# Ben-Bussch/Lunar_Module_Ascent_Trajectory_Optimiser

Measured on AMD Instinct MI355X. Metric: solved ascent NLPs/sec (N=200 collocation nodes), higher is better.
Workload: dtype f64; 1 GPU; BASELINE.json configs[2]: 4096-NLP Isp x dry-mass sweep (64x64, Isp 300-320 s, dry mass 2345-2545 kg), N=200 nodes, backward Euler (reference NODES=2), DCOST applied (the script's MV move penalty 1e-05, Launch_Optimiser.py:99, as an l1 term: the model the reference declares); move_penalty=True, batch_per_gpu=4096, global_batch=4096, n_nodes=200, parallelism=problem-sharded x1, gather only, converged=4096, of=4096

## Files before the change

### lunar_module_ascent_trajectory_optimiser_amd/csrc/ascent_persist.hip

```cpp
#include <hip/hip_runtime.h>

#pragma clang fp contract(on)

#include <cstdio>
#include <cstdlib>

#include "ascent.h"
#include "ascent_device.hpp"
#include "ascent_tile.hpp"
#include "ascent_persist.hpp"
#include "ascent_persist_dev.hpp"

using namespace ascent;

namespace {


ASC_DEV void start_move(double *w, int Kp, int k, double u, double up, bool warm, double dcw) {
  const double dl = u - up, eps = warm ? 1e-4 : 1e-2;
  w[(R_IT + O_LU) * Kp + k] = 0.0;
  w[(R_IT + O_PP) * Kp + k] = fmax(dl, 0.0) + eps;
  w[(R_IT + O_PN) * Kp + k] = fmax(-dl, 0.0) + eps;
  w[(R_IT + O_ZP) * Kp + k] = dcw;
  w[(R_IT + O_ZN) * Kp + k] = dcw;
// ... 354 lines not shown
    P.rd = fmax(P.rd, fmax(fabs(t.dcw - lu - kp.zpp), fabs(t.dcw + lu - kp.zpn)));
  }
  const double cs = SCHEME == 1 ? 0.5 * t.dt : t.dt;
  double fl[7], lt[7];
  ASC_UNROLL
  for (int i = 0; i < 7; i++) lt[i] = SCHEME == 1 ? l[i] + ln[i] : l[i];
  fzt_lambda<FORM>(kp.G, lt, fl);
  double r[7];
  ASC_UNROLL
  for (int i = 0; i < 7; i++) {
    r[i] = (FORM == 1 && i == IA) ? l[i] - cs * fl[i] : l[i] - cs * fl[i] - ln[i];
    P.rth -= t.hT * kp.F[i] * l[i];
    P.l1 += fabs(l[i]);
  }
  r[IA] += kp.dza;
  r[IM] += kp.dzm;
  if (k == K - 1) {
    const Scal &stt = t.stt;
    double z[7];
    ASC_UNROLL
    for (int i = 0; i < 7; i++) z[i] = in[(O_Z + i) * Kp + k];
    if constexpr (TERM == 2) {
      const Terminal tt = terminal_eval_any(d, z);
      double g4[4];
      terminal_grad_any(tt, stt.nu1, stt.nu2, g4);
      r[IX] += g4[0]; r[IY] += g4[1]; r[IVX] += g4[2]; r[IVY] += g4[3];
    } else {
      const Terminal tt = terminal_eval(d, z);
      r[IX] += stt.nu3 * tt.e3g[0] + stt.nu1 * tt.g1g[0];
      r[IY] += stt.nu3 * tt.e3g[1] + stt.nu1 * tt.g1g[1];
      r[IVX] += stt.nu3 * tt.e3g[2] + stt.nu2 * tt.g2g[0];
      r[IVY] += stt.nu3 * tt.e3g[3] + stt.nu2 * tt.g2g[1];
    }
  }
  ASC_UNROLL
  for (int i = 0; i < 7; i++) P.rd = fmax(P.rd, fabs(r[i]));
  double ruv = (FORM == 1 ? -0.5 * d.aub * l[IA] : -t.be * l[IW]) - kp.zb4 + kp.zb5;
  if constexpr (MP) ruv += lu - lun;
  P.rd = fmax(P.rd, fabs(ruv));
}

template <int SCHEME, int FORM, int MP = 0, int TERM = 0>
ASC_DEV void trial_node(const Der &d, int K, int Kp, int k, const NodeIn &n, const NodeIn &dn, const TrialCtx &t, bool live,
                        double *in, Part &P) {
  TrialKeep kp;
  trial_primal<SCHEME, FORM, MP, TERM>(d, K, Kp, k, n, dn, t, live, in, P, kp);
  double l[7], ln[7];
  ASC_UNROLL
  for (int i = 0; i < 7; i++) { l[i] = n.l[i] + t.alpha * dn.l[i]; ln[i] = n.ln[i] + t.alpha * dn.ln[i]; }
  const double lu = MP ? n.lu + t.alpha * dn.lu : 0.0, lun = MP ? n.lun + t.alpha * dn.lun : 0.0;
  trial_dual<SCHEME, FORM, MP, TERM>(d, K, Kp, k, kp, l, ln, lu, lun, t, live, in, P);
}


template <int SCHEME, int FORM, int MP = 0, int TERM = 0, int WIDE = 0>
__global__ __launch_bounds__(WAVE) void p_solve(const ascent_params *params, long batch, PGeo g, double *ws, int max_iter, double tol) {
  using L = Lay<MP>;
  constexpr int NS = L::NS, NIT = L::NIT, R_ST = L::R_ST, R_KA = L::R_KA, R_K0 = L::R_K0, NROWS = L::NROWS;
  constexpr int S_G = L::S_G, S_E = L::S_E, S_H = L::S_H, S_F = L::S_F, S_C = L::S_C, S_RZ = L::S_RZ, S_GT = L::S_GT, S_SC = L::S_SC;
  constexpr int RL = NS;
  static_assert(FORM == 0 || SCHEME == 0, "the v1 formulation is restated with backward Euler");
  __shared__ double stage[L::S_ROWS * LDW];
  __shared__ double outb[L::OUT_ROWS * LDW];
  __shared__ double lds_t[NPW][NS][NS];
  __shared__ double lds_d[NPW][3][8];
  __shared__ double lsc[NPW][NSCAL];
  __shared__ double lds_c[NPW][8];
  constexpr int CHN = WIDE ? 64 : CH;
  const int lane = threadIdx.x, grp = lane >> 4, role = lane & 15;
  const int nl = WIDE ? lane : role;
  const int cbase = WIDE ? 0 : grp * 16;
  const long p = WIDE ? (long)blockIdx.x : (long)blockIdx.x * NPW + grp;
  const bool live = p < batch;
  const long pc = live ? p : batch - 1;
  const int K = g.K, Kp = g.Kp, nch = g.nch;
  double *w = ws + (size_t)pc * g.nlp_doubles();
  double *gsc = w + (size_t)NROWS * Kp;
  double *sc = lsc[WIDE ? 0 : grp];
  const Der d = TERM == 2 ? derive_t(params[pc], 2) : derive(params[pc]);
  static_assert(TERM == 0 || (TERM == 2 && FORM == 0), "terminal 2 is carried for the current formulation");
  for (int r = role; r < NSCAL; r += 16) sc[r] = gsc[r];
  if (role < 8) lds_d[grp][2][role] = 0.0;
  wsync();
  if (!live && role == 0) sc[X_STATE] = ST_DONE;
  wsync();
  const int col = grp * 16 + role;
  const double hT = (1.0 / K) * d.T;
  constexpr int IB = FORM == 1 ? IA : IW;
  const double dcw = MP ? (FORM == 1 ? params[pc].dcost * 0.5 * d.aub : params[pc].dcost) : 0.0;
  constexpr double UINIT = FORM == 1 ? -1.0 : 0.0;

  PROF_DECL
  for (int round = 0; round < 64 * (max_iter + 2); round++) {
    PROF(9);
    int state = (int)sc[X_STATE];
    if (__all(state == ST_DONE)) break;
    if (state == ST_TRIAL) {
      const bool first = sc[X_FIRST] != 0.0;
      const double alpha = first ? 0.0 : sc[X_ALPHA], adu = first ? 0.0 : sc[X_ADU], mu = sc[X_MU];
      const Scal s = lds_scal(sc, X_S), ds = lds_scal(sc, X_D);
      const Scal stt = trial_scal(d, s, ds, alpha, adu, mu, first);
      const int cur = (int)sc[X_CUR];
      const double *ic = w + (size_t)(cur * NIT) * Kp, *stp = w + (size_t)R_ST * Kp;
      double *in = w + (size_t)((1 - cur) * NIT) * Kp;
      const double dt = hT * stt.th, be = dt * d.alpha;
      const double mlo = mu * 1e-10, mhi = mu * 1e10;
// ... 174 lines not shown
            const double dist[6] = {n.z[IA], d.aub - n.z[IA], n.z[IM], 1.0 - n.z[IM], n.u + 1.0, 1.0 - n.u};
            double id[6];
            ASC_UNROLL
            for (int b = 0; b < 6; b++) id[b] = rcp(dist[b]);
            H[7] += n.zb[0] * id[0] + n.zb[1] * id[1];
            H[9] += n.zb[2] * id[2] + n.zb[3] * id[3];
            ASC_UNROLL
            for (int i = 0; i < 8; i++) stage[(S_G + i) * LDW + col] = G[i];
            ASC_UNROLL
            for (int i = 0; i < 4; i++) stage[(S_E + i) * LDW + col] = E[i];
            ASC_UNROLL
            for (int i = 0; i < 10; i++) stage[(S_H + i) * LDW + col] = H[i];
            ASC_UNROLL
            for (int i = 0; i < 7; i++) {
              if (!MP || i != IM) stage[(S_F + i) * LDW + col] = hT * F[i];
              stage[(S_C + i) * LDW + col] = (FORM == 1 && i == IA) ? n.z[IA] - ha * (n.u + 1.0) : n.z[i] - n.zp[i] - dt * F[i];
              stage[(S_RZ + i) * LDW + col] = (FORM == 1 && i == IA) ? n.l[i] - cs * fl[i] : n.l[i] - cs * fl[i] - n.ln[i];
              stage[(S_GT + i) * LDW + col] = -hTc * fl[i];
            }
            const double scr[5] = {n.zb[4] * id[4] + n.zb[5] * id[5], FORM == 1 ? -ha * n.l[IA] : -be * n.l[IW], id[1] - id[0], id[3] - id[2],
                                   id[5] - id[4]};
            if constexpr (MP) {
              const MovePivot mvp = move_pivot(n.pp, n.pn, n.zpp, n.zpn, n.lu, dcw, mu, dw);
              stage[(S_C + 7) * LDW + col] = n.u - n.up - n.pp + n.pn;
              stage[(S_RZ + 7) * LDW + col] = (scr[1] + (n.lu - n.lun)) + mu * scr[4];
              stage[(S_GT + 7) * LDW + col] = FORM == 1 ? 0.0 : -hT * d.alpha * n.l[IW];
              stage[S_SC * LDW + col] = scr[0];
              stage[(S_SC + 1) * LDW + col] = mvp.Rd;
              stage[(S_SC + 2) * LDW + col] = mvp.gdl;
              stage[(S_RZ + IA) * LDW + col] += mu * scr[2];
              stage[(S_RZ + IM) * LDW + col] += mu * scr[3];
            } else {
              ASC_UNROLL
              for (int i = 0; i < 5; i++) stage[(S_SC + i) * LDW + col] = scr[i];
            }
          }
        }
        wsync();
        PROF(1);
        if (probe_rows) {
          const int k = c * CHN + nl;
          if (k < K && act && live) {
            ASC_UNROLL
            for (int i = 0; i < 8; i++) w[(size_t)(R_ST + i) * Kp + k] = stage[(S_G + i) * LDW + col];
            ASC_UNROLL
            for (int i = 0; i < 10; i++) w[(size_t)(R_ST + 8 + i) * Kp + k] = stage[(S_H + i) * LDW + col];
            ASC_UNROLL
            for (int i = 0; i < 7; i++) w[(size_t)(R_ST + 18 + i) * Kp + k] = stage[(S_C + i) * LDW + col];
          }
          wsync();
          continue;
        }
        if (act) {
          for (int jj = CHN - 1; jj >= 0; jj--) {
            const int k = c * CHN + jj;
            if (k >= K) continue;
            const int cj = cbase + jj;
            double gq[NS];
            ASC_UNROLL
            for (int i = 0; i < NS; i++) gq[i] = stage[grow[i] + cj];
            const double gA = stage[rowA + cj], gB = stage[rowB + cj];
            const double G[8] = {bcast16<0>(gA), bcast16<1>(gA), bcast16<2>(gA), bcast16<3>(gA),
                                 bcast16<4>(gA), bcast16<5>(gA), bcast16<6>(gA), bcast16<7>(gA)};
            const double E[4] = {bcast16<8>(gA), bcast16<9>(gA), bcast16<10>(gA), bcast16<11>(gA)};
            const double R0 = bcast16<12>(gA), ru0 = bcast16<13>(gA), bur = bcast16<14>(gA);
            const double bza = bcast16<15>(gA), bzm = bcast16<14>(gB);
            const double cc[8] = {bcast16<0>(gB), bcast16<1>(gB), bcast16<2>(gB), bcast16<3>(gB),
                                  bcast16<4>(gB), bcast16<5>(gB), bcast16<6>(gB), MP ? bcast16<15>(gB) : 0.0};
            const double rc1[7] = {bcast16<7>(gB), bcast16<8>(gB), bcast16<9>(gB), bcast16<10>(gB), bcast16<11>(gB),
                                   bcast16<12>(gB), MP ? hT * d.mrate : bcast16<13>(gB)};
            if (FORM == 1 && k < K - 1) {
              a[IA] = 0.0;
              if (role == IA) {
                ASC_UNROLL
                for (int i = 0; i < NS; i++) a[i] = 0.0;
              }
            }
            if (SCHEME == 1 && k < K - 1) {
              double t[7];
              fzt_lambda(G, a, t);
              ASC_UNROLL
              for (int i = 0; i < 7; i++) a[i] += cs * t[i];
              if (colr) {
                ASC_UNROLL
                for (int i = 0; i < NS; i++) lds_t[grp][role][i] = a[i];
                wsync();
                double r[NS];
                ASC_UNROLL
                for (int l2 = 0; l2 < NS; l2++) r[l2] = lds_t[grp][l2][role];
                fzt_lambda(G, r, t);
                ASC_UNROLL
                for (int i = 0; i < 7; i++) a[i] = r[i] + cs * t[i];
                if constexpr (MP) a[7] = r[7];
              }
              wsync();
            }
            ASC_UNROLL
            for (int i = 0; i < NS; i++) a[i] += gsgn[i] * gq[i];
            if constexpr (!MP) {
              a[IA] += bsc * bza;
              a[IM] += bsc * bzm;
            }
            if (dw != 0.0) {
              ASC_UNROLL
              for (int i = 0; i < NS; i++) a[i] += role == i ? dw : 0.0;
            }
            double b[NS];
            solveAT<FORM>(G, E, cs, a, b);
            if constexpr (MP) b[7] = a[7] + bu * b[IB];
            if (colr) {
              ASC_UNROLL
              for (int i = 0; i < NS; i++) lds_t[grp][role][i] = b[i];
              wsync();
              double t[NS];
              ASC_UNROLL
              for (int l2 = 0; l2 < NS; l2++) t[l2] = lds_t[grp][l2][role];
              solveAT<FORM>(G, E, cs, t, b);
              if constexpr (MP) b[7] = t[7] + bu * b[IB];
            }
            double mw[NS], D, coef;
            if constexpr (MP) {
              ASC_UNROLL
              for (int i = 0; i < NS; i++) mw[i] = bcast16<7>(b[i]);
              D = R0 + mw[7];
            } else {
              ASC_UNROLL
              for (int i = 0; i < NS; i++) mw[i] = bu * bcast16<IB>(b[i]);
              D = R0 + dw + bu * mw[IB];
            }
            const double iD = rcp(D);
            if constexpr (MP) {
              const double rsel = role == RL ? ru0 : 0.0;
              coef = (b[7] - rsel) * iD;
            } else {
              const double ru = ru0 + mu * bur, gu = FORM == 1 ? 0.0 : ru0 * ith;
              const double rsel = role == 7 ? ru : role == 8 ? gu : 0.0;
              coef = (bu * b[IB] - rsel) * iD;
            }
            ASC_UNROLL
            for (int i = 0; i < NS; i++) a[i] = b[i] - mw[i] * coef;
            outb[rowK + cj] = role < NS + 3 ? coef : D;
            if (colr) {
              double d0 = 0.0, d1 = 0.0;
              ASC_UNROLL
              for (int i = 0; i < NS; i++) {
                d0 -= a[i] * cc[i];
                if (i < 7) d1 += a[i] * rc1[i];
              }
              lds_d[grp][0][role] = d0;
              lds_d[grp][1][role] = d1;
            }
            wsync();
            {
              double prc[NS];
              ASC_UNROLL
              for (int i = 0; i < NS; i++) prc[i] = lds_d[grp][drow][i];
              double uu = 0.0, vv = 0.0;
              ASC_UNROLL
              for (int i = 0; i < NS; i++) {
                const double pj = a[i] - prc[i], sj = a[i] + pj;
                if (i < 7) uu += rc1[i] * sj;
                vv += cc[i] * sj;
                a[i] = pj;
              }
              U += uu; V += vv;
            }
          }
        }
        wsync();
        PROF(2);
        {
          const int k = c * CHN + nl;
          if (k < K && act) {
            if (live) {
              ASC_UNROLL
              for (int i = 0; i < NS + 3; i++) w[(size_t)(R_KA + i) * Kp + k] = outb[i * LDW + col];
            }
            const double k00 = outb[NS * LDW + col], k01 = outb[(NS + 1) * LDW + col], k02 = outb[(NS + 2) * LDW + col], D = outb[(NS + 3) * LDW + col];
            const double Dk1 = D * k01, Dk2 = D * k02;
            k10 += Dk1 * k00; k11 += Dk1 * k01; k12 += Dk1 * k02; k20 += Dk2 * k00; k22 += Dk2 * k02;
            if (!(D > 0.0)) bad = 1;
          }
        }
        wsync();
        PROF(3);
      }
      const double U0 = bcast16<RL>(U), U1 = bcast16<RL + 1>(U), V1 = bcast16<RL + 1>(V), U2 = bcast16<RL + 2>(U), V2 = bcast16<RL + 2>(V);
      k10 = gsumW<WIDE>(k10); k11 = gsumW<WIDE>(k11); k12 = gsumW<WIDE>(k12); k20 = gsumW<WIDE>(k20); k22 = gsumW<WIDE>(k22);
      bad = (int)gmaxW<WIDE>((double)bad);
      if (probe_rows) {
        if (act && role == 0) sc[X_STATE] = ST_DONE;
      } else if (act) {
        const double S10 = k10 + 0.5 * (U0 - V1), S11 = k11 + U1, S12 = k12 + 0.5 * U2, S20 = k20 - 0.5 * V2, S22 = k22;
        int ok = !bad;
        double dth = 0.0, dnu3 = 0.0;
        if (ok) {
          const double itl = rcp(s.th - d.tlb), itu = rcp(d.tub - s.th);
          const double rthp = sc[X_RTH] + mu * (itu - itl);
          const double sth = s.zlt * itl + s.zut * itu + dw;
          const double a11 = sth - S11, a12 = -S12, a22 = TERM == 2 ? -1.0 : -S22;
          const double b1 = -rthp + S10, b2 = -tm.e3 + S20;
          const double det = a11 * a22 - a12 * a12;
          if (det < 0.0) {
            const double idet = 1.0 / det;
            dth = (b1 * a22 - a12 * b2) * idet;
            dnu3 = (a11 * b2 - a12 * b1) * idet;
          } else {
            ok = 0;
          }
        }
        if (role == 0) {
          if (ok) {
            sc[X_DTH] = dth; sc[X_DNU3] = dnu3; sc[X_SIG1] = sig1; sc[X_SIG2] = sig2; sc[X_RS1] = rs1; sc[X_RS2] = rs2;
            sc[X_CG1] = tm.g1 - s.s1; sc[X_CG2] = tm.g2 - s.s2;
            sc[X_DWL] = dw; sc[X_STATE] = ST_FACTORED;
          } else {
            const double ndw = next_delta_w(dw, sc[X_DWL]);
            if (sc[X_PROBE] != 0.0) sc[X_STATE] = ST_DONE;
            else if (ndw > 1e10) { sc[X_STATUS] = ASCENT_REGULARISATION_FAILED; sc[X_STATE] = ST_DONE; }
// ... 105 lines not shown
            {
              double r[7];
              ASC_UNROLL
              for (int j = 0; j < 7; j++) r[j] = (j == IX ? 1.0 : 0.0) + cs * rvx[j];
              emit(IX, r, cs * rvx[IB]);
              ASC_UNROLL
              for (int j = 0; j < 7; j++) r[j] = (j == IY ? 1.0 : 0.0) + cs * rvy[j];
              emit(IY, r, cs * rvy[IB]);
              ASC_UNROLL
              for (int j = 0; j < 7; j++) r[j] = j == IA ? 1.0 : (j == IW && FORM == 0) ? cs : 0.0;
              emit(IA, r, FORM == 1 ? 1.0 : cs);
              ASC_UNROLL
              for (int j = 0; j < 7; j++) r[j] = j == IW ? 1.0 : 0.0;
              emit(IW, r, FORM == 1 ? 0.0 : 1.0);
            }
            if constexpr (MP) {
              double kj[7], v0;
              if (SCHEME == 1) {
                double t[7];
                fzt_lambda(Gp, ka, t);
                ASC_UNROLL
                for (int j = 0; j < 7; j++) kj[j] = ka[j] + cs * t[j];
                v0 = du00 - kj[IM] * dzm_p;
              } else {
                ASC_UNROLL
                for (int j = 0; j < 7; j++) kj[j] = ka[j];
                v0 = du00p;
              }
              ASC_UNROLL
              for (int j = 0; j < 6; j++) stage[(FS * 6 + j) * LDW + col] = (FORM == 1 && j == IA) ? 0.0 : -kj[j];
              stage[(FS * 6 + 6) * LDW + col] = 1.0 - ka[7];
              stage[(FS * 6 + NC) * LDW + col] = x0u + v0;
            } else if (SCHEME == 1) {
              double t[7];
              fzt_lambda(Gp, ka, t);
              ASC_UNROLL
              for (int j = 0; j < 6; j++) stage[(42 + j) * LDW + col] = -(ka[j] + cs * t[j]);
              stage[48 * LDW + col] = du00 - (ka[IM] + cs * t[IM]) * dzm_p;
            } else {
              ASC_UNROLL
              for (int j = 0; j < 6; j++) stage[(42 + j) * LDW + col] = (FORM == 1 && j == IA) ? 0.0 : -ka[j];
              stage[48 * LDW + col] = du00p;
            }
            outb[6 * LDW + col] = dzm_k;
          }
          wsync();
          PROF(4);
          if (act) {
            const int jn = min(CHN, K - c * CHN);
            for (int jj = 0; jj < jn; jj++) {
              const int cj = cbase + jj;
              const double *sj = stage + fbase + cj;
              const double m0 = sj[0], m1 = sj[LDW], m2 = sj[2 * LDW], m3 = sj[3 * LDW], m4 = sj[4 * LDW], m5 = sj[5 * LDW], vv = sj[NC * LDW];
              const double b0 = bcast16<0>(yown), b1 = bcast16<1>(yown), b2 = bcast16<2>(yown), b3 = bcast16<3>(yown),
                           b4 = bcast16<4>(yown), b5 = bcast16<5>(yown);
              const double e0 = (vv + m0 * b0) + m2 * b2, e1 = m1 * b1 + m3 * b3, e2 = m4 * b4 + m5 * b5;
              if constexpr (MP) {
                const double m6 = sj[6 * LDW], b6 = bcast16<6>(yown);
                yown = ((e0 + e1) + e2) + m6 * b6;
              } else {
                yown = (e0 + e1) + e2;
              }
              outb[fout + cj] = yown;
            }
          }
          wsync();
          PROF(5);
          if (kn < K && act) {
            double dzn[8];
            ASC_UNROLL
            for (int i = 0; i < 8; i++) dzn[i] = outb[i * LDW + col];
            const double id[6] = {rcp(a_), rcp(d.aub - a_), rcp(m_), rcp(1.0 - m_), rcp(u_ + 1.0), rcp(1.0 - u_)};
            const double dza = dzn[IA], dzm = dzn[IM], du = dzn[7];
            if (kn == K - 1) cpy<7>(dzK, dzn);
            ASC_FTBR(rmax, id[0], dza); ASC_FTBR(rmax, id[1], -dza);
            ASC_FTBR(rmax, id[2], dzm); ASC_FTBR(rmax, id[3], -dzm);
            ASC_FTBR(rmax, id[4], du); ASC_FTBR(rmax, id[5], -du);
            gsum += dza * (id[1] - id[0]) + dzm * (id[3] - id[2]) + du * (id[5] - id[4]);
            const double dx3[3] = {dza, dzm, du};
            double dzb[6];
            ASC_UNROLL
            for (int b = 0; b < 3; b++) {
              const double zl = zb[2 * b], zu = zb[2 * b + 1];
              dzb[2 * b] = id[2 * b] * (mu - zl * dx3[b]) - zl;
              dzb[2 * b + 1] = id[2 * b + 1] * (mu + zu * dx3[b]) - zu;
              ASC_FTB(adu, zl, dzb[2 * b]);
              ASC_FTB(adu, zu, dzb[2 * b + 1]);
            }
            if (live) {
              ASC_UNROLL
              for (int i = 0; i < 7; i++) stp[(O_Z + i) * Kp + kn] = dzn[i];
              stp[O_U * Kp + kn] = du;
              ASC_UNROLL
              for (int b = 0; b < 6; b++) stp[(O_ZB + b) * Kp + kn] = dzb[b];
            }
            if constexpr (MP) {
              const double du_p = nl > 0 ? outb[7 * LDW + col - 1] : carry_u;
              const double ddel = (du - du_p) - x0u;
              const MovePivot mvp = move_pivot(pp_, pn_, zpp_, zpn_, lu_, dcw, mu, dw);
              const double dlu = mvp.Rd * ddel + mvp.gdl;
              double dpp, dpn;
              if (mvp.sgp >= mvp.sgn) { dpp = (dlu - mvp.rp) * rcp(mvp.sgp); dpn = dpp - ddel; }
              else { dpn = (-dlu - mvp.rn) * rcp(mvp.sgn); dpp = ddel + dpn; }
              const double dzp = mvp.ip * (mu - zpp_ * dpp) - zpp_, dzn_ = mvp.in_ * (mu - zpn_ * dpn) - zpn_;
              ASC_FTBR(rmax, mvp.ip, dpp); ASC_FTBR(rmax, mvp.in_, dpn);
              ASC_FTB(adu, zpp_, dzp); ASC_FTB(adu, zpn_, dzn_);
              gsum -= dpp * mvp.ip + dpn * mvp.in_;
              gmove += dpp + dpn;
              clu -= x0u * (lu_ + dlu);
              if (live) {
                stp[O_LU * Kp + kn] = dlu; stp[O_PP * Kp + kn] = dpp; stp[O_PN * Kp + kn] = dpn; stp[O_ZP * Kp + kn] = dzp; stp[O_ZN * Kp + kn] = dzn_;
              }
// ... 102 lines not shown
              if constexpr (TERM == 2) terminal_hessian_any(QT, tm, s.nu1, s.nu2, sig1, sig2);
              else terminal_hessian(QT, tm, s.nu3, s.nu1, s.nu2, sig1, sig2);
              symv(QT, dz, qd);
              ASC_UNROLL
              for (int i = 0; i < 7; i++) r[i] -= qd[i];
              const double w1 = s.nu1 + sig1 * sc[X_CG1] + rs1, w2 = s.nu2 + sig2 * sc[X_CG2] + rs2;
              if constexpr (TERM == 2) {
                double g4[4];
                terminal_grad_any(tm, w1, w2, g4);
                r[IX] -= g4[0]; r[IY] -= g4[1]; r[IVX] -= g4[2]; r[IVY] -= g4[3];
              } else {
              r[IX] -= s.nu3 * tm.e3g[0] + w1 * tm.g1g[0] + tm.e3g[0] * dnu3;
              r[IY] -= s.nu3 * tm.e3g[1] + w1 * tm.g1g[1] + tm.e3g[1] * dnu3;
              r[IVX] -= s.nu3 * tm.e3g[2] + w2 * tm.g2g[0] + tm.e3g[2] * dnu3;
              r[IVY] -= s.nu3 * tm.e3g[3] + w2 * tm.g2g[1] + tm.e3g[3] * dnu3;
              }
            }
            double wv[7];
            solveAT<FORM>(G, E, cs, r, wv);
            {
              double rvx[7], rvy[7];
              ainv_vrows<FORM>(G, E, cs, rvx, rvy);
              ASC_UNROLL
              for (int i = 0; i < 7; i++) {
                double nr[7];
                nr[IVX] = rvx[i]; nr[IVY] = rvy[i];
                nr[IX] = (i == IX ? 1.0 : 0.0) + cs * rvx[i];
                nr[IY] = (i == IY ? 1.0 : 0.0) + cs * rvy[i];
                nr[IA] = FORM == 1 ? 0.0 : i == IA ? 1.0 : i == IW ? cs : 0.0;
                nr[IW] = i == IW ? 1.0 : 0.0;
                nr[IM] = i == IM ? 1.0 : 0.0;
                if (SCHEME == 1) {
                  double t[7];
                  fz_mul(G, nr, t);
                  ASC_UNROLL
                  for (int j = 0; j < 7; j++) nr[j] += cs * t[j];
                }
                ASC_UNROLL
                for (int j = 0; j < 5; j++) stage[(6 * i + j) * LDW + col] = nr[j];
              }
            }
            ASC_UNROLL
            for (int i = 0; i < 7; i++) stage[(6 * i + 5) * LDW + col] = wv[i];
            trial_primal<SCHEME, FORM, MP, TERM>(d, K, Kp, kn, n, dn, tc, live, in, P, kp);
          }
          wsync();
          PROF(7);
          if (act) {
            const int jj0 = min(CHN, K - c * CHN) - 1;
            for (int jj = jj0; jj >= 0; jj--) {
              const int cj = cbase + jj;
              const double *sj = stage + abase + cj;
              const double n0 = sj[0], n1 = sj[LDW], n2 = sj[2 * LDW], n3 = sj[3 * LDW], n4 = sj[4 * LDW], wv = sj[5 * LDW];
              const double b0 = bcast16<0>(lown), b1 = bcast16<1>(lown), b2 = bcast16<2>(lown), b3 = bcast16<3>(lown), b4 = bcast16<4>(lown);
              const double e0 = (wv + aself * lown) + n0 * b0, e1 = n1 * b1 + n2 * b2, e2 = n3 * b3 + n4 * b4;
              lown = (e0 + e1) + e2;
              outb[aout + cj] = lown;
            }
          }
          wsync();
          double dl[7], dln[7];
          if (kn < K && act) {
            ASC_UNROLL
            for (int i = 0; i < 7; i++) {
              dl[i] = outb[i * LDW + col];
              dln[i] = kn + 1 < K ? (nl < CHN - 1 ? outb[i * LDW + col + 1] : lds_c[WIDE ? 0 : grp][i]) : 0.0;
              ccl += ccn[i] * dl[i];
            }
            if (live) {
              ASC_UNROLL
              for (int i = 0; i < 7; i++) stp[(O_L + i) * Kp + kn] = dl[i];
            }
          }
          wsync();
          PROF(8);
          if (kn < K && act) {
            if (nl == 0) {
              ASC_UNROLL
              for (int i = 0; i < 7; i++) lds_c[WIDE ? 0 : grp][i] = dl[i];
            }
            double l[7], ln[7], lu = 0.0, lun = 0.0;
            ASC_UNROLL
            for (int i = 0; i < 7; i++) {
              l[i] = it[(O_L + i) * Kp + kn] + tc.alpha * dl[i];
              ln[i] = (kn + 1 < K ? it[(O_L + i) * Kp + kn + 1] : 0.0) + tc.alpha * dln[i];
            }
            if constexpr (MP) {
              lu = it[O_LU * Kp + kn] + tc.alpha * stp[O_LU * Kp + kn];
              lun = (kn + 1 < K ? it[O_LU * Kp + kn + 1] : 0.0) + tc.alpha * (kn + 1 < K ? stp[O_LU * Kp + kn + 1] : 0.0);
            }
            trial_dual<SCHEME, FORM, MP, TERM>(d, K, Kp, kn, kp, l, ln, lu, lun, tc, live, in, P);
          }
          PROF(0);
        }
        P.template reduceW<MP, WIDE>();
        ccl = gsumW<WIDE>(ccl);
        if (act) {
          cl += ccl;
          const Terminal &tm = tmK;
          double gd = MP ? mu * gsum + dcw * gmove : mu * gsum;
          if constexpr (MP) cl += clu;
          gd += ds.th * (1.0 - mu / dl_ + mu / dU) - mu * ds.s1 / s.s1 - mu * ds.s2 / s.s2;
          cl += tm.e3 * (s.nu3 + ds.nu3) + sc[X_CG1] * (s.nu1 + ds.nu1) + sc[X_CG2] * (s.nu2 + ds.nu2);
          const double c1 = sc[X_C1], slog = sc[X_SL];
          double nu_pen = sc[X_NUP];
          const double curv = -gd + cl;
          if (c1 > 0.0) {
            const double need = (gd + 0.5 * fmax(curv, 0.0)) / (0.9 * c1);
// ... 132 lines not shown
```

### lunar_module_ascent_trajectory_optimiser_amd/csrc/ascent_persist_dev.hpp

```cpp
#pragma once
#include <hip/hip_runtime.h>

#include "ascent.h"
#include "ascent_device.hpp"
#include "ascent_tile.hpp"

namespace {
using namespace ascent;

constexpr int NPW = 4, CH = 16;
constexpr int O_Z = 0, O_U = 7, O_L = 8, O_ZB = 15;
constexpr int O_LU = 21, O_PP = 22, O_PN = 23, O_ZP = 24, O_ZN = 25;
template <int MP>
struct Lay {
  static constexpr int NS = 7 + MP, NIT = 21 + 5 * MP;
  static constexpr int R_IT = 0, R_ST = 2 * NIT, R_KA = 3 * NIT, R_K0 = R_KA + NS, NROWS = R_K0 + 3;
  static constexpr int S_G = 0, S_E = 8, S_H = 12, S_F = 22, S_C = S_F + 7 - MP, S_RZ = S_C + NS, S_GT = S_RZ + NS, S_SC = S_GT + NS;
  static constexpr int S_ROWS = MP ? 56 : 55;
  static constexpr int OUT_ROWS = 11 + MP;
  static_assert(S_SC + (MP ? 3 : 5) <= S_ROWS, "stage rows");
};
constexpr int R_IT = 0;
constexpr int LDW = 65;
enum {
  X_STATE, X_ITERS, X_STATUS, X_CUR, X_FIRST, X_LS, X_MU, X_NUP, X_DW, X_DWL, X_ALPHA, X_ADU, X_PHI0, X_DM, X_C1, X_SL,
  X_RTH, X_DTH, X_DNU3, X_SIG1, X_SIG2, X_RS1, X_RS2, X_CG1, X_CG2,
  X_ITB,
  X_PROBE, X_PDW,
  X_TEVAL,
  X_P,
  X_PEND = X_P + 9,
  X_MV,
  X_S,
  X_D = X_S + 10,
  NSCAL = X_D + 10
};
constexpr int NSCAL_PAD = 64;
static_assert(NSCAL <= NSCAL_PAD, "scalar record");
enum { ST_TRIAL = 0, ST_FACTOR = 1, ST_FACTORED = 2, ST_DONE = 3 };

struct PGeo {
  int K, Kp, nch, form, mp, term, wide;
  __host__ __device__ int nit() const { return mp ? Lay<1>::NIT : Lay<0>::NIT; }
  __host__ __device__ int r_st() const { return 2 * nit(); }
  __host__ __device__ int nrows() const { return mp ? Lay<1>::NROWS : Lay<0>::NROWS; }
  __host__ __device__ size_t nlp_doubles() const { return (size_t)nrows() * Kp + NSCAL_PAD; }
};

template <int SRC>
ASC_DEV double bcast16(double v) {
  const long x = __builtin_amdgcn_mov_dpp(__builtin_bit_cast(long, v), 0x150 + SRC, 0xf, 0xf, false);
  return __builtin_bit_cast(double, x);
}
template <int N>
struct OneHot {
  double m[N];
  ASC_DEV explicit OneHot(int role) {
    ASC_UNROLL
    for (int i = 0; i < N; i++) m[i] = (role == i || (i == 0 && role >= N)) ? 1.0 : 0.0;
  }
  ASC_DEV double pick(const double *v) const {
    double r = m[0] * v[0];
    ASC_UNROLL
    for (int i = 1; i < N; i++) r += m[i] * v[i];
    return r;
  }
};
ASC_DEV void wsync() {
  __builtin_amdgcn_fence(__ATOMIC_RELEASE, "wavefront");
  __builtin_amdgcn_wave_barrier();
  __builtin_amdgcn_fence(__ATOMIC_ACQUIRE, "wavefront");
}
ASC_DEV double gsum16(double v) { v += __shfl_xor(v, 1); v += __shfl_xor(v, 2); v += __shfl_xor(v, 4); v += __shfl_xor(v, 8); return v; }
ASC_DEV double gmax16(double v) { v = fmax(v, __shfl_xor(v, 1)); v = fmax(v, __shfl_xor(v, 2)); v = fmax(v, __shfl_xor(v, 4)); return fmax(v, __shfl_xor(v, 8)); }
ASC_DEV double gmin16(double v) { v = fmin(v, __shfl_xor(v, 1)); v = fmin(v, __shfl_xor(v, 2)); v = fmin(v, __shfl_xor(v, 4)); return fmin(v, __shfl_xor(v, 8)); }
template <int WIDE> ASC_DEV double gsumW(double v) { v = gsum16(v); if constexpr (WIDE) { v += __shfl_xor(v, 16); v += __shfl_xor(v, 32); } return v; }
template <int WIDE> ASC_DEV double gmaxW(double v) { v = gmax16(v); if constexpr (WIDE) { v = fmax(v, __shfl_xor(v, 16)); v = fmax(v, __shfl_xor(v, 32)); } return v; }
template <int WIDE> ASC_DEV double gminW(double v) { v = gmin16(v); if constexpr (WIDE) { v = fmin(v, __shfl_xor(v, 16)); v = fmin(v, __shfl_xor(v, 32)); } return v; }

template <typename PT>
ASC_DEV Scal lds_scal(PT sc, int r0) {
  Scal s;
  s.th = sc[r0 + S_TH]; s.zlt = sc[r0 + S_ZLT]; s.zut = sc[r0 + S_ZUT]; s.s1 = sc[r0 + S_S1]; s.s2 = sc[r0 + S_S2];
  s.zs1 = sc[r0 + S_ZS1]; s.zs2 = sc[r0 + S_ZS2]; s.nu3 = sc[r0 + S_NU3]; s.nu1 = sc[r0 + S_NU1]; s.nu2 = sc[r0 + S_NU2];
  return s;
}
ASC_DEV void put_scal(double *sc, int r0, const Scal &s) {
  sc[r0 + S_TH] = s.th; sc[r0 + S_ZLT] = s.zlt; sc[r0 + S_ZUT] = s.zut; sc[r0 + S_S1] = s.s1; sc[r0 + S_S2] = s.s2;
  sc[r0 + S_ZS1] = s.zs1; sc[r0 + S_ZS2] = s.zs2; sc[r0 + S_NU3] = s.nu3; sc[r0 + S_NU1] = s.nu1; sc[r0 + S_NU2] = s.nu2;
}
ASC_DEV Scal trial_scal(const Der &d, const Scal &s, const Scal &ds, double alpha, double adu, double mu, bool first) {
  Scal t = s;
  if (first) return t;
  t.th += alpha * ds.th; t.s1 += alpha * ds.s1; t.s2 += alpha * ds.s2;
  t.nu3 += alpha * ds.nu3; t.nu1 += alpha * ds.nu1; t.nu2 += alpha * ds.nu2;
  t.zlt = clipz(s.zlt + adu * ds.zlt, t.th - d.tlb, mu);
  t.zut = clipz(s.zut + adu * ds.zut, d.tub - t.th, mu);
  t.zs1 = clipz(s.zs1 + adu * ds.zs1, t.s1, mu);
  t.zs2 = clipz(s.zs2 + adu * ds.zs2, t.s2, mu);
  return t;
}

struct NodeIn {
  double z[7], zp[7], l[7], ln[7], zb[6], u;
  double up, lu, lun, pp, pn, zpp, zpn;
};
// ... 54 lines not shown
```

Baseline: 645,200 NLPs/s.

## Fuse DPP broadcasts into FMAs and unroll serial Riccati sweep

Replaces separate DPP row broadcasts followed by multiplies with inline-asm v_fmac_f64_dpp using row_newbcast, in the backward sweep and the forward/adjoint recurrences. It adds a specialised solveAT/fzt that reads only the needed coefficients, makes the second solve and column dots unconditional across lanes to cut divergence, and unrolls the sweep loop by a configurable factor. The aim is fewer VALU instructions and fewer live registers on the latency-bound serial chain. Hand-written asm with DPP hazards (s_nop handling) risks correctness and limits compiler scheduling, and running the colr work on every lane adds redundant arithmetic.

```diff
diff --git a/lunar_module_ascent_trajectory_optimiser_amd/csrc/ascent_persist.hip b/lunar_module_ascent_trajectory_optimiser_amd/csrc/ascent_persist.hip
--- a/lunar_module_ascent_trajectory_optimiser_amd/csrc/ascent_persist.hip
+++ b/lunar_module_ascent_trajectory_optimiser_amd/csrc/ascent_persist.hip
@@ -430,6 +430,36 @@
   trial_dual<SCHEME, FORM, MP, TERM>(d, K, Kp, k, kp, l, ln, lu, lun, t, live, in, P);
 }
 
+
+#ifndef SWEEP_UNROLL
+#define SWEEP_UNROLL 2
+#endif
+struct SweepBlocks { double Gy[4], Ey[2]; };
+ASC_DEV SweepBlocks sweep_blocks(double gA) {
+  return {{bcast16<4>(gA), bcast16<5>(gA), bcast16<6>(gA), bcast16<7>(gA)}, {bcast16<10>(gA), bcast16<11>(gA)}};
+}
+template <int FORM>
+ASC_DEV void sweep_solveAT(double gA, const SweepBlocks &B, double dt, const double *r, double *v) {
+  const double t1 = r[IVX] + dt * r[IX], t2 = r[IVY] + dt * r[IY];
+  const double vvx = fmac_bc<8>(B.Ey[0] * t2, gA, t1), vvy = fmac_bc<9>(B.Ey[1] * t2, gA, t1);
+  const double va = r[IA] + dt * fmac_bc<2>(B.Gy[2] * vvy, gA, vvx);
+  v[IX] = r[IX] + dt * fmac_bc<0>(B.Gy[0] * vvy, gA, vvx);
+  v[IY] = r[IY] + dt * fmac_bc<1>(B.Gy[1] * vvy, gA, vvx);
+  v[IVX] = vvx;
+  v[IVY] = vvy;
+  v[IA] = va;
+  v[IM] = r[IM] + dt * fmac_bc<3>(B.Gy[3] * vvy, gA, vvx);
+  v[IW] = FORM == 1 ? r[IW] : r[IW] + dt * va;
+}
+ASC_DEV void sweep_fzt_lambda(double gA, const SweepBlocks &B, const double *l, double *fl) {
+  fl[IX] = fmac_bc<0>(B.Gy[0] * l[IVY], gA, l[IVX]);
+  fl[IY] = fmac_bc<1>(B.Gy[1] * l[IVY], gA, l[IVX]);
+  fl[IVX] = l[IX];
+  fl[IVY] = l[IY];
+  fl[IA] = fmac_bc<2>(B.Gy[2] * l[IVY], gA, l[IVX]);
+  fl[IW] = l[IA];
+  fl[IM] = fmac_bc<3>(B.Gy[3] * l[IVY], gA, l[IVX]);
+}
 
 template <int SCHEME, int FORM, int MP = 0, int TERM = 0, int WIDE = 0>
 __global__ __launch_bounds__(WAVE) void p_solve(const ascent_params *params, long batch, PGeo g, double *ws, int max_iter, double tol) {
@@ -710,23 +740,15 @@
           continue;
         }
         if (act) {
-          for (int jj = CHN - 1; jj >= 0; jj--) {
-            const int k = c * CHN + jj;
-            if (k >= K) continue;
-            const int cj = cbase + jj;
+          auto sweep_step = [&](const int jb, const int off) __attribute__((always_inline)) {
+            const int k = c * CHN + jb + off;
+            const int cj = cbase + jb;
             double gq[NS];
             ASC_UNROLL
-            for (int i = 0; i < NS; i++) gq[i] = stage[grow[i] + cj];
-            const double gA = stage[rowA + cj], gB = stage[rowB + cj];
-            const double G[8] = {bcast16<0>(gA), bcast16<1>(gA), bcast16<2>(gA), bcast16<3>(gA),
-                                 bcast16<4>(gA), bcast16<5>(gA), bcast16<6>(gA), bcast16<7>(gA)};
-            const double E[4] = {bcast16<8>(gA), bcast16<9>(gA), bcast16<10>(gA), bcast16<11>(gA)};
-            const double R0 = bcast16<12>(gA), ru0 = bcast16<13>(gA), bur = bcast16<14>(gA);
-            const double bza = bcast16<15>(gA), bzm = bcast16<14>(gB);
-            const double cc[8] = {bcast16<0>(gB), bcast16<1>(gB), bcast16<2>(gB), bcast16<3>(gB),
-                                  bcast16<4>(gB), bcast16<5>(gB), bcast16<6>(gB), MP ? bcast16<15>(gB) : 0.0};
-            const double rc1[7] = {bcast16<7>(gB), bcast16<8>(gB), bcast16<9>(gB), bcast16<10>(gB), bcast16<11>(gB),
-                                   bcast16<12>(gB), MP ? hT * d.mrate : bcast16<13>(gB)};
+            for (int i = 0; i < NS; i++) gq[i] = stage[grow[i] + cj + off];
+            const double gA = stage[rowA + cj + off], gB = stage[rowB + cj + off];
+            const SweepBlocks SB = sweep_blocks(gA);
+            const double R0 = bcast16<12>(gA), ru0 = bcast16<13>(gA);
             if (FORM == 1 && k < K - 1) {
               a[IA] = 0.0;
               if (role == IA) {
@@ -735,94 +757,104 @@
               }
             }
             if (SCHEME == 1 && k < K - 1) {
-              double t[7];
-              fzt_lambda(G, a, t);
+              double t[7], r[NS];
+              sweep_fzt_lambda(gA, SB, a, t);
+              ASC_UNROLL
+              for (int i = 0; i < NS; i++) r[i] = a[i];
               ASC_UNROLL
               for (int i = 0; i < 7; i++) a[i] += cs * t[i];
               if (colr) {
                 ASC_UNROLL
                 for (int i = 0; i < NS; i++) lds_t[grp][role][i] = a[i];
                 wsync();
-                double r[NS];
                 ASC_UNROLL
                 for (int l2 = 0; l2 < NS; l2++) r[l2] = lds_t[grp][l2][role];
-                fzt_lambda(G, r, t);
-                ASC_UNROLL
-                for (int i = 0; i < 7; i++) a[i] = r[i] + cs * t[i];
-                if constexpr (MP) a[7] = r[7];
               }
+              sweep_fzt_lambda(gA, SB, r, t);
+              ASC_UNROLL
+              for (int i = 0; i < 7; i++) a[i] = r[i] + cs * t[i];
+              if constexpr (MP) a[7] = r[7];
               wsync();
             }
             ASC_UNROLL
             for (int i = 0; i < NS; i++) a[i] += gsgn[i] * gq[i];
             if constexpr (!MP) {
-              a[IA] += bsc * bza;
-              a[IM] += bsc * bzm;
+              a[IA] = fmac_bc<15>(a[IA], gA, bsc);
+              a[IM] = fmac_bc<14>(a[IM], gB, bsc);
             }
             if (dw != 0.0) {
               ASC_UNROLL
               for (int i = 0; i < NS; i++) a[i] += role == i ? dw : 0.0;
             }
             double b[NS];
-            solveAT<FORM>(G, E, cs, a, b);
+            sweep_solveAT<FORM>(gA, SB, cs, a, b);
             if constexpr (MP) b[7] = a[7] + bu * b[IB];
             if (colr) {
               ASC_UNROLL
               for (int i = 0; i < NS; i++) lds_t[grp][role][i] = b[i];
               wsync();
-              double t[NS];
-              ASC_UNROLL
-              for (int l2 = 0; l2 < NS; l2++) t[l2] = lds_t[grp][l2][role];
-              solveAT<FORM>(G, E, cs, t, b);
-              if constexpr (MP) b[7] = t[7] + bu * b[IB];
-            }
-            double mw[NS], D, coef;
+              ASC_UNROLL
+              for (int l2 = 0; l2 < NS; l2++) a[l2] = lds_t[grp][l2][role];
+            }
+            sweep_solveAT<FORM>(gA, SB, cs, a, b);
+            if constexpr (MP) b[7] = a[7] + bu * b[IB];
+            double D, coef;
             if constexpr (MP) {
-              ASC_UNROLL
-              for (int i = 0; i < NS; i++) mw[i] = bcast16<7>(b[i]);
-              D = R0 + mw[7];
+              D = R0 + bcast16<7>(b[7]);
+              const double rsel = role == RL ? ru0 : 0.0;
+              coef = (b[7] - rsel) * rcp(D);
+              rank1_bc<7, NS>(b, coef);
+              ASC_UNROLL
+              for (int i = 0; i < NS; i++) a[i] = b[i];
             } else {
+              double mw[NS];
               ASC_UNROLL
               for (int i = 0; i < NS; i++) mw[i] = bu * bcast16<IB>(b[i]);
               D = R0 + dw + bu * mw[IB];
-            }
-            const double iD = rcp(D);
-            if constexpr (MP) {
-              const double rsel = role == RL ? ru0 : 0.0;
-              coef = (b[7] - rsel) * iD;
-            } else {
-              const double ru = ru0 + mu * bur, gu = FORM == 1 ? 0.0 : ru0 * ith;
+              const double ru = fmac_bc<14>(ru0, gA, mu), gu = FORM == 1 ? 0.0 : ru0 * ith;
               const double rsel = role == 7 ? ru : role == 8 ? gu : 0.0;
-              coef = (bu * b[IB] - rsel) * iD;
-            }
-            ASC_UNROLL
-            for (int i = 0; i < NS; i++) a[i] = b[i] - mw[i] * coef;
-            outb[rowK + cj] = role < NS + 3 ? coef : D;
-            if (colr) {
+              coef = (bu * b[IB] - rsel) * rcp(D);
+              ASC_UNROLL
+              for (int i = 0; i < NS; i++) a[i] = b[i] - mw[i] * coef;
+            }
+            outb[rowK + cj + off] = role < NS + 3 ? coef : D;
+            {
               double d0 = 0.0, d1 = 0.0;
-              ASC_UNROLL
-              for (int i = 0; i < NS; i++) {
-                d0 -= a[i] * cc[i];
-                if (i < 7) d1 += a[i] * rc1[i];
+              col_dots_bc<MP>(gB, a, d0, d1);
+              if constexpr (MP) d1 += a[6] * (hT * d.mrate);
+              if (colr) {
+                lds_d[grp][0][role] = d0;
+                lds_d[grp][1][role] = d1;
               }
-              lds_d[grp][0][role] = d0;
-              lds_d[grp][1][role] = d1;
             }
             wsync();
             {
-              double prc[NS];
+              double prc[NS], sj[NS];
               ASC_UNROLL
               for (int i = 0; i < NS; i++) prc[i] = lds_d[grp][drow][i];
-              double uu = 0.0, vv = 0.0;
               ASC_UNROLL
               for (int i = 0; i < NS; i++) {
-                const double pj = a[i] - prc[i], sj = a[i] + pj;
-                if (i < 7) uu += rc1[i] * sj;
-                vv += cc[i] * sj;
+                const double pj = a[i] - prc[i];
+                sj[i] = a[i] + pj;
                 a[i] = pj;
               }
+              double uu = 0.0, vv = 0.0;
+              uu = fmac_bc<7>(uu, gB, sj[0]); uu = fmac_bc<8>(uu, gB, sj[1]); uu = fmac_bc<9>(uu, gB, sj[2]); uu = fmac_bc<10>(uu, gB, sj[3]);
+              uu = fmac_bc<11>(uu, gB, sj[4]); uu = fmac_bc<12>(uu, gB, sj[5]);
+              if constexpr (MP) uu += (hT * d.mrate) * sj[6];
+              else uu = fmac_bc<13>(uu, gB, sj[6]);
+              vv = fmac_bc<0>(vv, gB, sj[0]); vv = fmac_bc<1>(vv, gB, sj[1]); vv = fmac_bc<2>(vv, gB, sj[2]); vv = fmac_bc<3>(vv, gB, sj[3]);
+              vv = fmac_bc<4>(vv, gB, sj[4]); vv = fmac_bc<5>(vv, gB, sj[5]); vv = fmac_bc<6>(vv, gB, sj[6]);
+              if constexpr (MP) vv = fmac_bc<15>(vv, gB, sj[7]);
               U += uu; V += vv;
             }
+          };
+          int jj = min(CHN - 1, K - 1 - c * CHN);
+          static_assert(SWEEP_UNROLL == 1 || SWEEP_UNROLL == 2 || SWEEP_UNROLL == 4, "SWEEP_UNROLL");
+          for (; (jj + 1) % SWEEP_UNROLL != 0; jj--) sweep_step(jj, 0);
+          for (; jj >= 0; jj -= SWEEP_UNROLL) {
+            ASC_UNROLL
+            for (int u = SWEEP_UNROLL - 1; u >= 0; u--) sweep_step(jj - (SWEEP_UNROLL - 1), u);
           }
         }
         wsync();
@@ -1034,12 +1066,12 @@
               const int cj = cbase + jj;
               const double *sj = stage + fbase + cj;
               const double m0 = sj[0], m1 = sj[LDW], m2 = sj[2 * LDW], m3 = sj[3 * LDW], m4 = sj[4 * LDW], m5 = sj[5 * LDW], vv = sj[NC * LDW];
-              const double b0 = bcast16<0>(yown), b1 = bcast16<1>(yown), b2 = bcast16<2>(yown), b3 = bcast16<3>(yown),
-                           b4 = bcast16<4>(yown), b5 = bcast16<5>(yown);
-              const double e0 = (vv + m0 * b0) + m2 * b2, e1 = m1 * b1 + m3 * b3, e2 = m4 * b4 + m5 * b5;
+              const double b3 = bcast16<3>(yown), b5 = bcast16<5>(yown);
+              const double e0 = fmac_bc<2>(fmac_bc_after<0>(vv, yown, m0, b3), yown, m2);
+              const double e1 = fmac_bc<1>(m3 * b3, yown, m1), e2 = fmac_bc<4>(m5 * b5, yown, m4);
               if constexpr (MP) {
-                const double m6 = sj[6 * LDW], b6 = bcast16<6>(yown);
-                yown = ((e0 + e1) + e2) + m6 * b6;
+                const double m6 = sj[6 * LDW];
+                yown = fmac_bc<6>((e0 + e1) + e2, yown, m6);
               } else {
                 yown = (e0 + e1) + e2;
               }
@@ -1248,8 +1280,8 @@
               const int cj = cbase + jj;
               const double *sj = stage + abase + cj;
               const double n0 = sj[0], n1 = sj[LDW], n2 = sj[2 * LDW], n3 = sj[3 * LDW], n4 = sj[4 * LDW], wv = sj[5 * LDW];
-              const double b0 = bcast16<0>(lown), b1 = bcast16<1>(lown), b2 = bcast16<2>(lown), b3 = bcast16<3>(lown), b4 = bcast16<4>(lown);
-              const double e0 = (wv + aself * lown) + n0 * b0, e1 = n1 * b1 + n2 * b2, e2 = n3 * b3 + n4 * b4;
+              const double b2 = bcast16<2>(lown), b4 = bcast16<4>(lown);
+              const double e0 = fmac_bc_after<0>(wv + aself * lown, lown, n0, b2), e1 = fmac_bc<1>(n2 * b2, lown, n1), e2 = fmac_bc<3>(n4 * b4, lown, n3);
               lown = (e0 + e1) + e2;
               outb[aout + cj] = lown;
             }
diff --git a/lunar_module_ascent_trajectory_optimiser_amd/csrc/ascent_persist_dev.hpp b/lunar_module_ascent_trajectory_optimiser_amd/csrc/ascent_persist_dev.hpp
--- a/lunar_module_ascent_trajectory_optimiser_amd/csrc/ascent_persist_dev.hpp
+++ b/lunar_module_ascent_trajectory_optimiser_amd/csrc/ascent_persist_dev.hpp
@@ -52,6 +52,56 @@
   const long x = __builtin_amdgcn_mov_dpp(__builtin_bit_cast(long, v), 0x150 + SRC, 0xf, 0xf, false);
   return __builtin_bit_cast(double, x);
 }
+template <int SRC, bool VALU_SRC = false>
+ASC_DEV double fmac_bc(double acc, double v, double b) {
+  if constexpr (VALU_SRC)
+    asm("s_nop 1\n\tv_fmac_f64_dpp %0, %1, %2 row_newbcast:%3 row_mask:0xf bank_mask:0xf" : "+v"(acc) : "v"(v), "v"(b), "n"(SRC));
+  else
+    asm("v_fmac_f64_dpp %0, %1, %2 row_newbcast:%3 row_mask:0xf bank_mask:0xf" : "+v"(acc) : "v"(v), "v"(b), "n"(SRC));
+  return acc;
+}
+template <int SRC>
+ASC_DEV double fmac_bc_after(double acc, double v, double b, double after) {
+  asm("v_fmac_f64_dpp %0, %1, %2 row_newbcast:%3 row_mask:0xf bank_mask:0xf" : "+v"(acc) : "v"(v), "v"(b), "n"(SRC), "v"(after));
+  return acc;
+}
+template <int SRC, bool VALU_SRC = false>
+ASC_DEV double fnmac_bc(double acc, double v, double b) {
+  if constexpr (VALU_SRC)
+    asm("s_nop 1\n\tv_fmac_f64_dpp %0, -%1, %2 row_newbcast:%3 row_mask:0xf bank_mask:0xf" : "+v"(acc) : "v"(v), "v"(b), "n"(SRC));
+  else
+    asm("v_fmac_f64_dpp %0, -%1, %2 row_newbcast:%3 row_mask:0xf bank_mask:0xf" : "+v"(acc) : "v"(v), "v"(b), "n"(SRC));
+  return acc;
+}
+template <int SRC, int N>
+ASC_DEV void rank1_bc(double *x, double c) {
+  static_assert(N == 7 || N == 8, "rank1_bc");
+#define ASC_R1(i_) "\n\tv_fmac_f64_dpp %" #i_ ", -%" #i_ ", %[c] row_newbcast:%[s] row_mask:0xf bank_mask:0xf"
+  if constexpr (N == 8)
+    asm("s_nop 1" ASC_R1(0) ASC_R1(1) ASC_R1(2) ASC_R1(3) ASC_R1(4) ASC_R1(5) ASC_R1(6) ASC_R1(7)
+        : "+v"(x[0]), "+v"(x[1]), "+v"(x[2]), "+v"(x[3]), "+v"(x[4]), "+v"(x[5]), "+v"(x[6]), "+v"(x[7]) : [c] "v"(c), [s] "n"(SRC));
+  else
+    asm("s_nop 1" ASC_R1(0) ASC_R1(1) ASC_R1(2) ASC_R1(3) ASC_R1(4) ASC_R1(5) ASC_R1(6)
+        : "+v"(x[0]), "+v"(x[1]), "+v"(x[2]), "+v"(x[3]), "+v"(x[4]), "+v"(x[5]), "+v"(x[6]) : [c] "v"(c), [s] "n"(SRC));
+#undef ASC_R1
+}
+template <int MP>
+ASC_DEV void col_dots_bc(double g, const double *a, double &d0, double &d1) {
+#define ASC_D0(l_, i_) "v_fmac_f64_dpp %[d0], -%[g], %[a" #i_ "] row_newbcast:" #l_ " row_mask:0xf bank_mask:0xf\n\t"
+#define ASC_D1(l_, i_) "v_fmac_f64_dpp %[d1], %[g], %[a" #i_ "] row_newbcast:" #l_ " row_mask:0xf bank_mask:0xf\n\t"
+  if constexpr (MP)
+    asm(ASC_D0(0, 0) ASC_D1(7, 0) ASC_D0(1, 1) ASC_D1(8, 1) ASC_D0(2, 2) ASC_D1(9, 2) ASC_D0(3, 3) ASC_D1(10, 3) ASC_D0(4, 4) ASC_D1(11, 4)
+        ASC_D0(5, 5) ASC_D1(12, 5) ASC_D0(6, 6) ASC_D0(15, 7)
+        : [d0] "+v"(d0), [d1] "+v"(d1)
+        : [g] "v"(g), [a0] "v"(a[0]), [a1] "v"(a[1]), [a2] "v"(a[2]), [a3] "v"(a[3]), [a4] "v"(a[4]), [a5] "v"(a[5]), [a6] "v"(a[6]), [a7] "v"(a[7]));
+  else
+    asm(ASC_D0(0, 0) ASC_D1(7, 0) ASC_D0(1, 1) ASC_D1(8, 1) ASC_D0(2, 2) ASC_D1(9, 2) ASC_D0(3, 3) ASC_D1(10, 3) ASC_D0(4, 4) ASC_D1(11, 4)
+        ASC_D0(5, 5) ASC_D1(12, 5) ASC_D0(6, 6) ASC_D1(13, 6)
+        : [d0] "+v"(d0), [d1] "+v"(d1)
+        : [g] "v"(g), [a0] "v"(a[0]), [a1] "v"(a[1]), [a2] "v"(a[2]), [a3] "v"(a[3]), [a4] "v"(a[4]), [a5] "v"(a[5]), [a6] "v"(a[6]));
+#undef ASC_D0
+#undef ASC_D1
+}
 template <int N>
 struct OneHot {
   double m[N];
```

Result: no change. 645,600 NLPs/s (median of 2 runs) (+0.1%).
